# benjiebob/SMALify

Measured on AMD Instinct MI355X. Metric: fitter iterations/sec, higher is better.
Workload: dtype f32

## Files before the change

smalify_amd/csrc/kernels_lbs_backward.inc:

```

__global__ void __launch_bounds__(256)
vertex_bwd_kernel(ModelDev m, int M, const float* __restrict__ proj, const float* __restrict__ dface,
                  const float* __restrict__ dJ41 ,
                  const float* __restrict__ dverts_ext ,
                  const float* __restrict__ Am, float* __restrict__ dvert ,
                  float* __restrict__ dvp , float* __restrict__ dtr_part ) {
  __shared__ float As[420];
  __shared__ float dJs[123];
  __shared__ float red[16];
  const int Vp = m.Vp;
  PHASE_MARK(pv0);
  int n, vblock;
  xcd_block(Vp / 256, n, vblock);
  if (n >= M) return;
  const int v = vblock * 256 + threadIdx.x;
  constexpr int kPre = 8;
  const int vc = min(v, m.V - 1);
  const int vf0 = m.vf_off[vc], vf1 = (v < m.V) ? m.vf_off[vc + 1] : vf0;
  int vfi[kPre];
#pragma unroll
  for (int q = 0; q < kPre; ++q) vfi[q] = m.vf_idx[min(vf0 + q, max(vf1 - 1, vf0))];
  for (int i = threadIdx.x; i < 420; i += 256) As[i] = Am[(size_t)n * 420 + i];
  for (int i = threadIdx.x; i < 123; i += 256) dJs[i] = dJ41 ? dJ41[(size_t)n * 123 + i] : 0.f;
  __syncthreads();
// ... 110 lines not shown
  const int ncol = 3 * m.Vp;
  const int c = bx * 256 + threadIdx.x;
  float g = 0.f;
  if (c < ncol) {
    if (shared) {
      const int per = (M + gzn - 1) / gzn;
      const int n0 = bz * per, n1 = min(M, n0 + per);
      double gd = 0.0;
#pragma unroll 8
      for (int n = n0; n < n1; ++n) gd += (double)dvp[(size_t)n * ncol + c];
      g = (float)gd;
    } else {
      g = dvp[(size_t)by * ncol + c];
    }
  }
  const size_t pidx = (size_t)by * gzn * gx + (size_t)bz * gx + bx;
  const int lane = threadIdx.x & 63, w = threadIdx.x >> 6;
  for (int b0 = 0; b0 < nb; b0 += 32) {
    float val[32];
    const int cc = min(c, ncol - 1);
#pragma unroll
    for (int b = 0; b < 32; ++b) val[b] = m.sd[(size_t)min(b0 + b, nb - 1) * ncol + cc];
#pragma unroll
    for (int b = 0; b < 32; ++b) val[b] = (c < ncol && b0 + b < nb) ? g * val[b] : 0.f;
    const float tot = wave_sums<32>(val, lane);
    __syncthreads();
    if ((lane & 1) == 0) part[w][lane >> 1] = tot;
    __syncthreads();
    if (threadIdx.x < 32 && b0 + threadIdx.x < nb)
      dbeta_part[pidx * nb + b0 + threadIdx.x] = ((part[0][threadIdx.x] + part[1][threadIdx.x]) + part[2][threadIdx.x]) + part[3][threadIdx.x];
  }
}

constexpr int PBM_SPLITS = 24, PBM_U = 2, PBM_TILES = 4;
static_assert(PBM_SPLITS % 8 == 0, "the blocks of a column split are placed on one XCD (ids in chunks of 8 splits)");
__device__ __forceinline__ void
poseblend_bwd_mfma_block(const ModelDev& m, int M, int tchunk, int kpair, int split, const float* __restrict__ dvp,
                         float* __restrict__ dpf_part , float (*red)[8][64]) {
  const int lane = threadIdx.x & 63, w = threadIdx.x >> 6;
  const int ncol = 3 * m.Vp, nsteps = ncol / 16;
  const int per = (nsteps + PBM_SPLITS * 4 - 1) / (PBM_SPLITS * 4);
  const int s_beg = (split * 4 + w) * per, s_end = min(nsteps, s_beg + per);
  const int nft = (M + 15) / 16, t0 = tchunk * PBM_TILES, nt = min(PBM_TILES, nft - t0);
  const int k0 = kpair * 32;
  const int row = lane & 15, cq = (lane >> 4) * 4;
  const float4* pa[PBM_TILES];
#pragma unroll
  for (int t = 0; t < PBM_TILES; ++t)
    pa[t] = reinterpret_cast<const float4*>(dvp + (size_t)min((t0 + t) * 16 + row, M - 1) * ncol + cq);
  const float4* pb0 = reinterpret_cast<const float4*>(m.pd + (size_t)min(k0 + row, 305) * ncol + cq);
  const float4* pb1 = reinterpret_cast<const float4*>(m.pd + (size_t)min(k0 + 16 + row, 305) * ncol + cq);
  f32x4 acc0[PBM_TILES], acc1[PBM_TILES];
#pragma unroll
  for (int t = 0; t < PBM_TILES; ++t) { acc0[t] = f32x4{0.f, 0.f, 0.f, 0.f}; acc1[t] = acc0[t]; }
  for (int st0 = s_beg; st0 < s_end; st0 += PBM_U) {
    float4 B0[PBM_U], B1[PBM_U], A[PBM_TILES][PBM_U];
#pragma unroll
    for (int u = 0; u < PBM_U; ++u) {
      const int st = min(st0 + u, nsteps - 1);
      B0[u] = pb0[st * 4]; B1[u] = pb1[st * 4];
#pragma unroll
      for (int t = 0; t < PBM_TILES; ++t) {
        A[t][u] = make_float4(0.f, 0.f, 0.f, 0.f);
        if (t < nt && st0 + u < s_end) A[t][u] = pa[t][st * 4];
      }
    }
    __builtin_amdgcn_sched_barrier(0);
#pragma unroll
    for (int u = 0; u < PBM_U; ++u) {
#pragma unroll
      for (int t = 0; t < PBM_TILES; ++t) {
        if (t < nt) {
          acc0[t] = __builtin_amdgcn_mfma_f32_16x16x4f32(A[t][u].x, B0[u].x, acc0[t], 0, 0, 0);
          acc1[t] = __builtin_amdgcn_mfma_f32_16x16x4f32(A[t][u].x, B1[u].x, acc1[t], 0, 0, 0);
          acc0[t] = __builtin_amdgcn_mfma_f32_16x16x4f32(A[t][u].y, B0[u].y, acc0[t], 0, 0, 0);
          acc1[t] = __builtin_amdgcn_mfma_f32_16x16x4f32(A[t][u].y, B1[u].y, acc1[t], 0, 0, 0);
          acc0[t] = __builtin_amdgcn_mfma_f32_16x16x4f32(A[t][u].z, B0[u].z, acc0[t], 0, 0, 0);
          acc1[t] = __builtin_amdgcn_mfma_f32_16x16x4f32(A[t][u].z, B1[u].z, acc1[t], 0, 0, 0);
          acc0[t] = __builtin_amdgcn_mfma_f32_16x16x4f32(A[t][u].w, B0[u].w, acc0[t], 0, 0, 0);
          acc1[t] = __builtin_amdgcn_mfma_f32_16x16x4f32(A[t][u].w, B1[u].w, acc1[t], 0, 0, 0);
        }
      }
    }
    __builtin_amdgcn_sched_barrier(0);
  }
#pragma unroll
  for (int t = 0; t < PBM_TILES; ++t) {
    if (t < nt) {
#pragma unroll
      for (int r = 0; r < 4; ++r) { red[w][r][lane] = acc0[t][r]; red[w][4 + r][lane] = acc1[t][r]; }
      __syncthreads();
#pragma unroll
      for (int q = 0; q < 2; ++q) {
        const int reg = w * 2 + q, r = reg & 3, tile = reg >> 2;
        const float tot = ((red[0][reg][lane] + red[1][reg][lane]) + red[2][reg][lane]) + red[3][reg][lane];
        const int n = (t0 + t) * 16 + 4 * (lane >> 4) + r, k = k0 + tile * 16 + (lane & 15);
        if (n < M && k < 306) dpf_part[((size_t)split * M + n) * 308 + k] = tot;
      }
      __syncthreads();
    }
  }
}

__host__ __device__ inline int mid_pb_ids(int M) { return 10 * PBM_SPLITS * (((M + 15) / 16 + PBM_TILES - 1) / PBM_TILES); }
__host__ __device__ inline int mid_da_ids(int M) { return xcd_grid(35, M); }
__host__ __device__ inline int mid_grid(int M, int nPB) { return (nPB ? mid_pb_ids(M) : 0) + mid_da_ids(M); }
__global__ void __launch_bounds__(256, 4)
lbs_bwd_mid_kernel(ModelDev m, int M, int nPB, const float* __restrict__ dvert, const float* __restrict__ vposed,
                   const float* __restrict__ dvp, float* __restrict__ dA, float* __restrict__ dpf_part) {
  __shared__ float part[4][32];
  __shared__ float tile_red[4][8][64];
  int blk = blockIdx.x;
  if (nPB > 0) {
    const int ids = mid_pb_ids(M);
    if (blk < ids) {
      PHASE_MARK(pm0);
      const int tchunk = blk / (10 * PBM_SPLITS), r = blk - tchunk * (10 * PBM_SPLITS);
      const int chunk = r / 80, q = r - chunk * 80;
      poseblend_bwd_mfma_block(m, M, tchunk, q >> 3, chunk * 8 + (q & 7), dvp, dpf_part, tile_red);
      PHASE_MARK(pm1);
      PHASE_END(PH_MID_PB, pm0, pm1);
      return;
    }
    blk -= ids;
  }
  PHASE_MARK(pd0);
  int n, j;
  xcd_block_of(blk, 35, n, j);
  if (n >= M) return;
  dA_block(m, j, n, dvert, vposed, dA, part);
  PHASE_MARK(pd1); PHASE_END(PH_MID_DA, pd0, pd1);
}

__global__ void __launch_bounds__(256)
chain_bwd_kernel(ModelDev m, int M, const float* __restrict__ theta, const float* __restrict__ Rm,
                 const float* __restrict__ Gm, const float* __restrict__ scm,
                 const float* __restrict__ Jrest, int j_stride, const float* __restrict__ dA,
                 const float* __restrict__ dpf_part, int CS, const float* __restrict__ dth_direct,
                 float* __restrict__ dtheta , float* __restrict__ dls ,
                 float* __restrict__ dJrest , float* __restrict__ dbetaJ ,
                 float* __restrict__ dRs_out ,
                 int nb, int betas_shared, int nDB_x, int nDB_y, int nDB_z, const float* __restrict__ dvp,
                 float* __restrict__ dbeta_part ) {
  PHASE_MARK(pc0);
  if ((int)blockIdx.x >= M) {
    __shared__ float rpart[4][32];
    const int blk = (int)blockIdx.x - M;
    dbeta_block(m, M, nb, betas_shared, blk % nDB_x, (blk / nDB_x) % nDB_y, blk / (nDB_x * nDB_y), nDB_x, nDB_z, dvp, dbeta_part, rpart);
    PHASE_MARK(pcr);
    PHASE_END(PH_CHAIN_RIDER, pc0, pcr);
    return;
  }
  __shared__ float R[35][9], G[35][12], sc[35][3], J[35][3];
  __shared__ float dG[35][12], dR[35][9], dJ[35][3];
  __shared__ float cG[35][12], cJ[35][3], cS[35][3], sOwn[35][3];
  __shared__ float dRp[35][9], djv[35][3];
  __shared__ int sidx[105];
  __shared__ float psum[4][320];
  __shared__ float isc[35][3];
  __shared__ float sJS[105 * 48];
  __shared__ float dAs[35][12];
  __shared__ unsigned char t_lvl_off[36], t_lvl_joint[36], t_child_off[36], t_child_idx[36], t_par[36];
  __shared__ uint2 t_sch[kTreeMaxPass][8];
  const int n = blockIdx.x, l = threadIdx.x;
  const TreeLevels& tl = m.tree;
  if (l < 36) {
    t_lvl_off[l] = tl.lvl_off[l]; t_child_off[l] = tl.child_off[l];
    if (l < 35) { t_lvl_joint[l] = tl.lvl_joint[l]; t_child_idx[l] = tl.child_idx[l]; t_par[l] = (unsigned char)max(m.parents[l], 0); }
  }
  if (l >= 128 && l < 128 + kTreeMaxPass * 8) {
    const int q = l - 128;
    const unsigned char* ch = tl.pass_child[q >> 3][q & 7];
    t_sch[q >> 3][q & 7] = make_uint2((unsigned)tl.pass_joint[q >> 3][q & 7] | ((unsigned)tl.pass_parent[q >> 3][q & 7] << 8) | ((unsigned)tl.pass_nchild[q >> 3][q & 7] << 16),
                                      (unsigned)ch[0] | ((unsigned)ch[1] << 8) | ((unsigned)ch[2] << 16) | ((unsigned)ch[3] << 24));
  }
  const int lth = min(l, 34);
  const float th_pre[3] = {theta[((size_t)n * 35 + lth) * 3], theta[((size_t)n * 35 + lth) * 3 + 1], theta[((size_t)n * 35 + lth) * 3 + 2]};
  float dthd_pre[3] = {0.f, 0.f, 0.f};
  if (dth_direct) {
#pragma unroll
    for (int a = 0; a < 3; ++a) dthd_pre[a] = dth_direct[(size_t)n * 105 + lth * 3 + a];
  }
  const int nlev = tl.nlev;
  const bool js_lds = dbetaJ && m.NBall <= 48;
  const int njs = js_lds ? 105 * m.NBall : 1;
  float js_tmp[20];
  const float* js_src = js_lds ? m.JS : Rm + (size_t)n * 315;
#pragma unroll
  for (int r = 0; r < 20; ++r) js_tmp[r] = js_src[min(l + 256 * r, njs - 1)];
  {
    const int l2 = l + 256;
    const float r0v = Rm[(size_t)n * 315 + l], r1v = Rm[(size_t)n * 315 + min(l2, 314)];
    const float g0v = Gm[(size_t)n * 420 + l], g1v = Gm[(size_t)n * 420 + min(l2, 419)];
    const float a0v = dA[(size_t)n * 420 + l], a1v = dA[(size_t)n * 420 + min(l2, 419)];
    const int lc = min(l, 104);
    const float sv = scm[(size_t)n * 105 + lc], jv = Jrest[(size_t)n * j_stride + lc];
    const int siv = m.scale_idx[lc];
    constexpr int kMaxPer = (PBM_SPLITS + 3) / 4;
    const int per = (CS + 3) / 4, qd = l >> 6, c0 = qd * per, c1 = min(CS, c0 + per);
    const size_t stride = (size_t)M * 308;
    float pv[5][kMaxPer];
    const bool fast = dpf_part != nullptr && per <= kMaxPer;
    if (fast) {
#pragma unroll
      for (int r = 0; r < 5; ++r) {
        const float* src = dpf_part + (size_t)n * 308 + min((l & 63) + 64 * r, 305);
#pragma unroll
        for (int c = 0; c < kMaxPer; ++c) pv[r][c] = src[(size_t)min(c0 + c, CS - 1) * stride];
      }
    }
    if (js_lds) {
#pragma unroll
      for (int r = 0; r < 20; ++r) { const int i = l + 256 * r; if (i < njs) sJS[i] = js_tmp[r]; }
    }
    R[l / 9][l % 9] = r0v;
    if (l2 < 315) R[l2 / 9][l2 % 9] = r1v;
    G[l / 12][l % 12] = g0v; dAs[l / 12][l % 12] = a0v;
    if (l2 < 420) { G[l2 / 12][l2 % 12] = g1v; dAs[l2 / 12][l2 % 12] = a1v; }
    if (l < 105) {
      sc[l / 3][l % 3] = sv; isc[l / 3][l % 3] = 1.0f / sv;
      J[l / 3][l % 3] = jv;
      sOwn[l / 3][l % 3] = 0.f; cS[l / 3][l % 3] = 0.f; cJ[l / 3][l % 3] = 0.f;
      sidx[l] = siv;
    }
    if (dpf_part) {
#pragma unroll
      for (int r = 0; r < 5; ++r) {
        const int el = (l & 63) + 64 * r;
        if (el < 306) {
          float sacc = 0.f;
          if (fast) {
            if (c0 < c1) sacc = pv[r][0];
#pragma unroll
            for (int c = 1; c < kMaxPer; ++c)
              if (c0 + c < c1) sacc += pv[r][c];
          } else {
            const float* src = dpf_part + (size_t)n * 308 + el;
            for (int c = c0; c < c1; ++c) sacc += src[c * stride];
          }
          psum[qd][el] = sacc;
        }
      }
    }
  }
  __syncthreads();
  PHASE_MARK(pc1);
  for (int i = l; i < 315; i += 256)
    dR[i / 9][i % 9] = (i >= 9 && dpf_part) ? ((psum[0][i - 9] + psum[1][i - 9]) + psum[2][i - 9]) + psum[3][i - 9] : 0.f;
  for (int i = l; i < 420; i += 256) {
    const int j = i / 12, e = i % 12, a = e >> 2, b = e & 3;
    const float* da = dAs[j];
    dG[j][e] = (b < 3) ? da[e] - da[a * 4 + 3] * J[j][b] : da[e];
  }
  for (int i = l; i < 105; i += 256) {
    const int j = i / 3, c = i % 3;
    const float* da = dAs[j];
    dJ[j][c] = -(G[j][0 * 4 + c] * da[3] + G[j][1 * 4 + c] * da[7] + G[j][2 * 4 + c] * da[11]);
  }
  __syncthreads();
  PHASE_MARK(pc2);
  const int slot = l / 12, e = l % 12;
  if (l < 64 && tl.fast) {
    const int npass = tl.npass;
    const int slot_c = min(slot, 7);
    uint2 sch_n = t_sch[max(npass - 1, 0)][slot_c];
#pragma unroll 1
    for (int k = npass - 1; k >= 0; --k) {
      const uint2 sch = sch_n;
      sch_n = t_sch[max(k - 1, 0)][slot_c];
      const bool live = (sch.x & 255u) != 255u;
      const int i = live ? (int)(sch.x & 255u) : 0, p = live ? (int)((sch.x >> 8) & 255u) : 0, nch = live ? (int)(sch.x >> 16) : 0;
      const unsigned chil_k = sch.y;
      if (live) {
        float acc = dG[i][e];
        float cv[kTreeMaxChildren];
#pragma unroll
        for (int q = 0; q < kTreeMaxChildren; ++q) cv[q] = cG[(chil_k >> (8 * q)) & 255u][e];
#pragma unroll
        for (int q = 0; q < kTreeMaxChildren; ++q) acc += (q < nch) ? cv[q] : 0.f;
        dG[i][e] = acc;
      }
      __builtin_amdgcn_fence(__ATOMIC_ACQ_REL, "wavefront");
      __builtin_amdgcn_wave_barrier();
      if (live) {
        if (e < 9) {
          const int a = e / 3, b = e % 3;
          dRp[i][e] = G[p][0 * 4 + a] * dG[i][0 * 4 + b] + G[p][1 * 4 + a] * dG[i][1 * 4 + b] + G[p][2 * 4 + a] * dG[i][2 * 4 + b];
        } else {
          const int a = e - 9;
          djv[i][a] = G[p][0 * 4 + a] * dG[i][3] + G[p][1 * 4 + a] * dG[i][7] + G[p][2 * 4 + a] * dG[i][11];
        }
      }
      __builtin_amdgcn_fence(__ATOMIC_ACQ_REL, "wavefront");
      __builtin_amdgcn_wave_barrier();
      if (live) {
        if (e < 9) {
          const int a = e / 3, c = e % 3;
          float acc = dG[i][a * 4 + 3] * (J[i][c] - J[p][c]);
#pragma unroll
          for (int b = 0; b < 3; ++b) acc = fmaf(dG[i][a * 4 + b], R[i][c * 3 + b] * sc[i][b] * isc[p][c], acc);
          cG[i][a * 4 + c] = acc;
          dR[i][a * 3 + c] += dRp[i][a * 3 + c] * sc[i][c] * isc[p][a];
        } else {
          const int a = e - 9;
          cG[i][a * 4 + 3] = dG[i][a * 4 + 3];
          cJ[i][a] = djv[i][a];
          {
            const int b = a;
            float acc = 0.f;
#pragma unroll
            for (int r = 0; r < 3; ++r) acc = fmaf(dRp[i][r * 3 + b], R[i][r * 3 + b] * isc[p][r], acc);
            sOwn[i][b] = acc;
          }
          {
            float acc = 0.f;
#pragma unroll
            for (int b = 0; b < 3; ++b) acc = fmaf(dRp[i][a * 3 + b], R[i][a * 3 + b] * sc[i][b] * isc[p][a], acc);
            cS[i][a] = acc * isc[p][a];
          }
        }
      }
      __builtin_amdgcn_fence(__ATOMIC_ACQ_REL, "wavefront");
      __builtin_amdgcn_wave_barrier();
    }
  } else if (l < 64)
  for (int L = nlev - 1; L >= 1; --L) {
    const int j0 = t_lvl_off[L], nj = t_lvl_off[L + 1] - j0;
    for (int base = 0; base < nj; base += 5) {
      const bool live = (slot < 5) && (base + slot < nj);
      const int i = live ? t_lvl_joint[j0 + base + slot] : 0;
      const int p = live ? t_par[i] : 0;
      if (live) {
        float acc = dG[i][e];
        for (int q = t_child_off[i]; q < t_child_off[i + 1]; ++q) acc += cG[t_child_idx[q]][e];
        dG[i][e] = acc;
      }
      __builtin_amdgcn_fence(__ATOMIC_ACQ_REL, "workgroup");
      __builtin_amdgcn_wave_barrier();
      if (live) {
        if (e < 9) {
          const int a = e / 3, b = e % 3;
          dRp[i][e] = G[p][0 * 4 + a] * dG[i][0 * 4 + b] + G[p][1 * 4 + a] * dG[i][1 * 4 + b] + G[p][2 * 4 + a] * dG[i][2 * 4 + b];
        } else {
          const int a = e - 9;
          djv[i][a] = G[p][0 * 4 + a] * dG[i][3] + G[p][1 * 4 + a] * dG[i][7] + G[p][2 * 4 + a] * dG[i][11];
        }
      }
      __builtin_amdgcn_fence(__ATOMIC_ACQ_REL, "workgroup");
      __builtin_amdgcn_wave_barrier();
      if (live) {
        if (e < 9) {
          const int a = e / 3, c = e % 3;
          float acc = dG[i][a * 4 + 3] * (J[i][c] - J[p][c]);
#pragma unroll
          for (int b = 0; b < 3; ++b) acc = fmaf(dG[i][a * 4 + b], R[i][c * 3 + b] * sc[i][b] * isc[p][c], acc);
          cG[i][a * 4 + c] = acc;
          dR[i][a * 3 + c] += dRp[i][a * 3 + c] * sc[i][c] * isc[p][a];
        } else {
          const int a = e - 9;
          cG[i][a * 4 + 3] = dG[i][a * 4 + 3];
          cJ[i][a] = djv[i][a];
          {
            const int b = a;
            float acc = 0.f;
#pragma unroll
            for (int r = 0; r < 3; ++r) acc = fmaf(dRp[i][r * 3 + b], R[i][r * 3 + b] * isc[p][r], acc);
            sOwn[i][b] = acc;
          }
          {
            float acc = 0.f;
#pragma unroll
            for (int b = 0; b < 3; ++b) acc = fmaf(dRp[i][a * 3 + b], R[i][a * 3 + b] * sc[i][b] * isc[p][a], acc);
            cS[i][a] = acc * isc[p][a];
          }
        }
      }
      __builtin_amdgcn_fence(__ATOMIC_ACQ_REL, "workgroup");
      __builtin_amdgcn_wave_barrier();
    }
  }
  __syncthreads();
  PHASE_MARK(pc3);
  if (l < 12) {
    float acc = dG[0][l];
    for (int q = t_child_off[0]; q < t_child_off[1]; ++q) acc += cG[t_child_idx[q]][l];
    dG[0][l] = acc;
  }
  __syncthreads();
  if (l < 9) dR[0][l] += dG[0][(l / 3) * 4 + (l % 3)];
  for (int i = l; i < 105; i += 256) {
    const int j = i / 3, a = i % 3;
    float aj = dJ[j][a], as = 0.f;
    for (int q = t_child_off[j]; q < t_child_off[j + 1]; ++q) { aj -= cJ[t_child_idx[q]][a]; as -= cS[t_child_idx[q]][a]; }
    if (j > 0) { aj += cJ[j][a]; as += sOwn[j][a]; }
    else aj += dG[0][a * 4 + 3];
    dJ[j][a] = aj;
    sOwn[j][a] = as;
  }
  __syncthreads();
  PHASE_MARK(pc4);
  if (l < 35) {
    const float th[3] = {th_pre[0], th_pre[1], th_pre[2]};
    float g[9], d[3];
#pragma unroll
    for (int q = 0; q < 9; ++q) g[q] = dR[l][q];
    if (dRs_out) {
#pragma unroll
      for (int q = 0; q < 9; ++q) dRs_out[((size_t)n * 35 + l) * 9 + q] = g[q];
    }
    rodrigues_bwd(th, g, d);
#pragma unroll
    for (int a = 0; a < 3; ++a)
      dtheta[(size_t)n * 105 + l * 3 + a] = d[a] + (dth_direct ? dthd_pre[a] : 0.f);
  }
  if (dls) {
    const int w = l >> 6, lane = l & 63;
    for (int sidx_l = w; sidx_l < 6; sidx_l += 4) {
      float v = 0.f;
      if (sidx[lane] == sidx_l) v = sOwn[lane / 3][lane % 3] * sc[lane / 3][lane % 3];
      if (lane + 64 < 105 && sidx[lane + 64] == sidx_l) v += sOwn[(lane + 64) / 3][(lane + 64) % 3] * sc[(lane + 64) / 3][(lane + 64) % 3];
      v = wave_sum(v);
      if (lane == 0) dls[(size_t)n * 6 + sidx_l] = v;
    }
  }
  for (int i = l; i < 105; i += 256) dJrest[(size_t)n * 105 + i] = dJ[i / 3][i % 3];
  if (dbetaJ) {
    const int w = l >> 6, b = l & 63;
    if (b < m.NBall) {
      float acc = 0.f;
      if (js_lds) {
#pragma unroll 9
        for (int r = 0; r < 27; ++r) { const int i = w * 27 + r; if (i < 105) acc = fmaf(dJ[i / 3][i % 3], sJS[i * m.NBall + b], acc); }
      } else {
        for (int i = w * 27; i < min(105, w * 27 + 27); ++i) acc = fmaf(dJ[i / 3][i % 3], m.JS[i * m.NBall + b], acc);
      }
      psum[w][b] = acc;
    }
    __syncthreads();
    if (l < m.NBall) dbetaJ[(size_t)n * m.NBall + l] = ((psum[0][l] + psum[1][l]) + psum[2][l]) + psum[3][l];
  }
  PHASE_MARK(pc5);
  PHASE_ADD(PH_CHAIN, 0, pc0, pc1); PHASE_ADD(PH_CHAIN, 1, pc1, pc2); PHASE_ADD(PH_CHAIN, 2, pc2, pc3); PHASE_ADD(PH_CHAIN, 3, pc3, pc4); PHASE_ADD(PH_CHAIN, 4, pc4, pc5);
  PHASE_END(PH_CHAIN, pc0, pc5);
}

template <bool kPerImage>
__global__ void __launch_bounds__(256)
assemble_kernel(AssembleArgs a, AssembleExt x) {
  __shared__ float red[16];
  __shared__ double bsum[12][32];
  __shared__ float part[32][8];
  __shared__ double dpart[32][8];
  __shared__ int is_last;
  const int t = threadIdx.x;
  PHASE_MARK(pa0);
  const int M = a.M;
  const int nbs = a.betas_shared ? 1 : M;
  int role = blockIdx.x;
  const int ph_role = (role < nbs) ? PH_ASM_BETA : PH_ASM_ELEM;
  if (role < nbs) {
    if (a.g_betas) {
      const int s = role;
      for (int b0 = 0; b0 < a.nb; b0 += 20) {
        if (b0) __syncthreads();
        BetaOperands bo;
        asm_beta_fetch(a, s, b0, bo);
        asm_beta_slices(a, s, b0, bo, bsum);
        __syncthreads();
        const float tot = asm_beta_total(a, s, b0, bo, bsum);
        if constexpr (kPerImage) {
          if (t < 20 && b0 + t < a.nb) a.g_betas[s * a.nb + b0 + t] = x.gb_prior_pf ? tot + x.gb_prior_pf[(size_t)s * x.gb_stride + b0 + t] : tot;
        } else
        if (t < 20 && b0 + t < a.nb) a.g_betas[s * a.nb + b0 + t] = tot;
      }
    }
  } else if ((role -= nbs) == 0) {
    if (a.g_ls) {
      if (a.ls_shared) {
        LsOperands lo;
        asm_ls_fetch(a, lo);
        asm_ls_slices(a, lo, dpart);
        __syncthreads();
        const float tot = asm_ls_total(a, lo, dpart);
        if (t < 6) a.g_ls[t] = tot;
      } else {
        if (kPerImage && x.gls_prior_pf)
          for (int i = t; i < M * 6; i += 256) a.g_ls[i] = a.dls[i] + x.gls_prior_pf[(size_t)(i / 6) * x.gls_stride + i % 6];
        else
          for (int i = t; i < M * 6; i += 256) a.g_ls[i] = a.dls[i];
      }
    }
  } else if ((role -= 1) < kAsmElem) {
    const int gt = role * 256 + t, gs = kAsmElem * 256;
    for (int i = gt; i < M * 3; i += gs) {
      const int n = i / 3, e = i % 3;
      if (a.g_grot) a.g_grot[i] = asm_grot_elem(a, n, e);
      if (a.g_trans) a.g_trans[i] = asm_trans_elem(a, n, e);
    }
    if (a.g_jrot) {
      const int total = M * 102;
      for (int i0 = gt; i0 < total; i0 += 8 * gs) {
        float v[8];
#pragma unroll
        for (int u = 0; u < 8; ++u) {
          const int i = min(i0 + u * gs, total - 1), n = i / 102, e = i % 102;
          v[u] = asm_jrot_elem(a, n, e);
        }
#pragma unroll
        for (int u = 0; u < 8; ++u)
          if (i0 + u * gs < total) a.g_jrot[i0 + u * gs] = v[u];
      }
    }
  } else if (a.losses) {
    role -= kAsmElem;
    float lsil = 0.f;
    if (a.tile_loss) {
      for (int k = role * 256 + t; k < M * a.T; k += kAsmLoss * 256) {
        const int n = k / a.T;
        const int Bn = frame_window_size(n, a.win);
        lsil += a.tile_loss[k] * (a.w_sil / ((float)Bn * (float)a.S * (float)a.S));
      }
    }
    long long qs = 0;
    if (a.qloss) for (int k = role * 256 + t; k < a.nqblk; k += kAsmLoss * 256) qs += a.qloss[k];
    qs = wave_sum_i64(qs);
    __shared__ long long qred[4];
    if ((t & 63) == 0) qred[t >> 6] = qs;
    lsil = block_sum(lsil, red);
    if (t == 0) { a.lpart[role] = lsil; a.qpart[role] = (qred[0] + qred[1]) + (qred[2] + qred[3]); }
  }
  PHASE_MARK(pa1);
  PHASE_END(ph_role, pa0, pa1);
  (void)ph_role;
  if (!a.losses) return;
  __threadfence();
  __syncthreads();
  if (t == 0) is_last = (atomicAdd(a.counter, 1) == (int)gridDim.x - 1);
  __syncthreads();
  if (!is_last) return;
  __threadfence();
  static_assert(kAsmLoss == 16, "butterfly below");
  float lsil = 0.f;
  if (t < 64) {
    const volatile float* lp = a.lpart;
    lsil = (t < kAsmLoss) ? lp[t] : 0.f;
#pragma unroll
    for (int o = 8; o > 0; o >>= 1) lsil += __shfl_xor(lsil, o, 64);
// ... 262 lines not shown
```

smalify_amd/csrc/kernels_lbs_forward.inc:

```

constexpr int kAsmFr = 8, kAsmPa = 32, kAsmLs = 4;
struct BetaOperands { float fv[kAsmFr], pv[kAsmPa], prior; };
__device__ __forceinline__ void asm_beta_fetch(const AssembleArgs& a, int s, int b0, BetaOperands& o) {
  const int t = threadIdx.x, slice = min(t / 20, 11), b = min(b0 + t % 20, a.nb - 1);
  const int nlo = a.betas_shared ? 0 : s, nhi = a.betas_shared ? a.M : s + 1, nparts = a.nblk_beta * a.ngrp_beta;
  const float* pj = a.dbetaJ + b;
  const float* pp = a.dbeta_part + (size_t)s * nparts * a.nb + b;
#pragma unroll
  for (int u = 0; u < kAsmFr; ++u) o.fv[u] = pj[(size_t)min(nlo + slice + 12 * u, nhi - 1) * a.NBall];
#pragma unroll
  for (int u = 0; u < kAsmPa; ++u) o.pv[u] = pp[(size_t)min(slice + 12 * u, nparts - 1) * a.nb];
  o.prior = (a.gb_prior && s == 0) ? a.gb_prior[min(b0 + min(t, 19), a.nb - 1)] : 0.f;
}
__device__ __forceinline__ void asm_beta_slices(const AssembleArgs& a, int s, int b0, BetaOperands& o, double (*bsum)[32]) {
  const int t = threadIdx.x, bl = t % 20, slice = t / 20, b = b0 + bl;
  if (slice < 12 && b < a.nb) {
    const int nlo = a.betas_shared ? 0 : s, nhi = a.betas_shared ? a.M : s + 1, nparts = a.nblk_beta * a.ngrp_beta;
    const float* pj = a.dbetaJ + b;
    const float* pp = a.dbeta_part + (size_t)s * nparts * a.nb + b;
    double acc = 0.0;
    for (int n0 = nlo + slice; n0 < nhi; n0 += 12 * kAsmFr) {
#pragma unroll
      for (int u = 0; u < kAsmFr; ++u)
        if (n0 + 12 * u < nhi) acc += (double)o.fv[u];
// ... 56 lines not shown
}
__device__ __forceinline__ float asm_theta_elem(const AssembleArgs& a, int n, int l) {
  const float* mk = (l < 3) ? a.gmask + l : a.rmask + max(l - 3, 0);
  return a.dtheta[(size_t)n * 105 + l] * *mk;
}
__device__ __forceinline__ float asm_grot_elem(const AssembleArgs& a, int n, int e) { return asm_theta_elem(a, n, e); }
__device__ __forceinline__ float asm_jrot_elem(const AssembleArgs& a, int n, int e) { return asm_theta_elem(a, n, 3 + e); }
__device__ __forceinline__ float asm_trans_elem(const AssembleArgs& a, int n, int e) {
  double acc = a.dtr_direct ? (double)a.dtr_direct[n * 3 + e] : 0.0;
#pragma unroll 16
  for (int vt = 0; vt < a.nvt; ++vt) acc += (double)a.dtr_part[((size_t)vt * a.M + n) * 3 + e];
  return (float)acc;
}


struct HeadArgs {
  int M, Mp, nb, betas_stride, ls_stride, nshape_x, nshape, prior_D, prior_use_ls;
  const float* betas;
  const float* theta_in;
  const float* grot;
  const float* jrot;
  const float* gmask;
  const float* rmask;
  const float* logscale;
  float* theta;
  float* Jrest;
  float* v_shaped;
  float *Rm, *Gm, *scm, *Am, *pfT;
  const float* prior_prec;
  const float* prior_mean;
  float prior_w;
  float *prior_loss, *prior_gb, *prior_gls;
  const float* Rs_in;
  const float* joff;
  int joff_stride;
  const float* voff;
};

constexpr int kPendingNb = 20;
struct HeadShared {
  float beta[kPendingNb], ls[8], grot[4];
  double bsum[12][32], dpart[32][8];
};
struct AdamOperands { float p, m, v; };
__device__ __forceinline__ AdamOperands pending_load(const PendingStep& p, const PendingTensor& T, int i) {
  return AdamOperands{T.p_in[i], p.fresh ? 0.f : T.m_in[i], p.fresh ? 0.f : T.v_in[i]};
}
__device__ __forceinline__ float pending_adam(const PendingStep& p, const PendingTensor& T, int i, const AdamOperands& o, float gi, bool store) {
  float mi, vi, pv = o.p;
  adam_update(gi, o.m, o.v, p.b1, p.b2, p.eps, p.step_size, p.bc2_sqrt, mi, vi, pv);
  if (store) { T.m[i] = mi; T.v[i] = vi; T.p[i] = pv; T.g[i] = gi; }
  return pv;
}
struct SharedOperands { AdamOperands beta, ls; BetaOperands bo; LsOperands lo; };
__device__ __forceinline__ void pending_shared_fetch(const PendingStep& p, const HeadArgs& a, int n, SharedOperands& o) {
  const int t = threadIdx.x;
  o.beta = pending_load(p, p.betas, min(t, 19));
  if (p.betas.train) asm_beta_fetch(p.g, 0, 0, o.bo);
  if (a.logscale) {
    if (p.g.ls_shared) o.ls = pending_load(p, p.ls, min(t, 5));
    else if (!p.ls.train) o.ls.p = a.logscale[(size_t)n * a.ls_stride + min(t, 5)];
    if (p.ls.train && p.g.ls_shared) asm_ls_fetch(p.g, o.lo);
  }
}
__device__ __forceinline__ void pending_shared_slices(const PendingStep& p, SharedOperands& o, HeadShared& sh) {
  if (p.betas.train) asm_beta_slices(p.g, 0, 0, o.bo, sh.bsum);
  if (p.ls.train && p.g.ls_shared) asm_ls_slices(p.g, o.lo, sh.dpart);
}
__device__ __forceinline__ void pending_shared_step(const PendingStep& p, const HeadArgs& a, const SharedOperands& o, HeadShared& sh) {
  const int t = threadIdx.x;
  const bool store = blockIdx.x == 0;
  if (p.betas.train) {
    const float gi = asm_beta_total(p.g, 0, 0, o.bo, sh.bsum);
    if (t < 20) sh.beta[t] = pending_adam(p, p.betas, t, o.beta, gi, store);
  } else if (t < 20) {
    sh.beta[t] = o.beta.p;
  }
  if (a.logscale && (p.g.ls_shared || !p.ls.train)) {
    if (p.ls.train) {
      const float gi = asm_ls_total(p.g, o.lo, sh.dpart);
      if (t < 6) sh.ls[t] = pending_adam(p, p.ls, t, o.ls, gi, store);
    } else if (t < 6) {
      sh.ls[t] = o.ls.p;
    }
  }
}
struct ThetaOperands { AdamOperands ao; float gi; };
__device__ __forceinline__ void pending_jrot_fetch(const PendingStep& p, int n, ThetaOperands& o) {
  const int l = max(min((int)threadIdx.x, 104), 3);
  o.ao = pending_load(p, p.jrot, n * 102 + (l - 3));
  o.gi = asm_theta_elem(p.g, n, l);
}
__device__ __forceinline__ float pending_jrot_step(const PendingStep& p, int n, const ThetaOperands& o) {
  const int l = threadIdx.x;
  if (l >= 3 && l < 105 && p.jrot.train) return pending_adam(p, p.jrot, n * 102 + (l - 3), o.ao, o.gi, true);
  return o.ao.p;
}
__device__ __forceinline__ void pending_frame_extras(const PendingStep& p, int n, HeadShared& sh) {
  const int l = threadIdx.x;
  if (l >= 128 && l < 131) {
    const int i = n * 3 + (l - 128);
    if (p.trans.train) pending_adam(p, p.trans, i, pending_load(p, p.trans, i), asm_trans_elem(p.g, n, l - 128), true);
  } else if (l >= 224 && l < 227) {
    const int i = n * 3 + (l - 224);
    const AdamOperands ao = pending_load(p, p.grot, i);
    sh.grot[l - 224] = p.grot.train ? pending_adam(p, p.grot, i, ao, asm_theta_elem(p.g, n, l - 224), true) : ao.p;
  } else if (l >= 192 && l < 198) {
    if (p.ls.train && !p.g.ls_shared) { const int i = n * 6 + (l - 192); sh.ls[l - 192] = pending_adam(p, p.ls, i, pending_load(p, p.ls, i), p.g.dls[i], true); }
  }
}

template <bool kPending>
__device__ __forceinline__ void
pose_block(const ModelDev& m, const HeadArgs& a, int n, const PendingStep* pend, HeadShared* sh) {
  __shared__ float th[105];
  __shared__ float R[35][9];
  __shared__ float sc[35][3], isc[35][3];
  __shared__ __attribute__((aligned(16))) float G[35][12];
  __shared__ float J[35][3];
  __shared__ unsigned char t_lvl_off[36], t_lvl_joint[36], t_par[36];
  __shared__ unsigned char t_pj[kTreeMaxPass][8], t_pp[kTreeMaxPass][8];
  const int l = threadIdx.x, M = a.M;
  PHASE_MARK(ph0);
  const TreeLevels& tl = m.tree;
  if (l < 36) {
    t_lvl_off[l] = tl.lvl_off[l];
    if (l < 35) { t_lvl_joint[l] = tl.lvl_joint[l]; t_par[l] = (unsigned char)max(m.parents[l], 0); }
  }
  if (l >= 128 && l < 128 + kTreeMaxPass * 8) { const int q = l - 128; t_pj[q >> 3][q & 7] = tl.pass_joint[q >> 3][q & 7]; t_pp[q >> 3][q & 7] = tl.pass_parent[q >> 3][q & 7]; }
  const int nlev = tl.nlev;
  float tv_pend = 0.f, js_pre[kPendingNb], jt_pre = 0.f, mv_pre = 0.f;
  int idx_pre = 0;
  if constexpr (kPending) {
    const int lc = min(l, 104);
    idx_pre = m.scale_idx[lc]; jt_pre = m.Jt[lc];
    mv_pre = (lc < 3) ? a.gmask[lc] : a.rmask[max(lc - 3, 0)];
#pragma unroll
    for (int b = 0; b < kPendingNb; ++b) js_pre[b] = m.JS[lc * m.NBall + b];
    SharedOperands so;
    ThetaOperands to;
    pending_shared_fetch(*pend, a, n, so);
    pending_jrot_fetch(*pend, n, to);
    pending_frame_extras(*pend, n, *sh);
    tv_pend = pending_jrot_step(*pend, n, to);
    pending_shared_slices(*pend, so, *sh);
    PHASE_MARK(pp1);
    __syncthreads();
    pending_shared_step(*pend, a, so, *sh);
    PHASE_MARK(pp2);
    __syncthreads();
    if (l < 3) tv_pend = sh->grot[l];
    PHASE_MARK(pp3);
    PHASE_ADD(PH_HEAD_POSE, 4, ph0, pp1); PHASE_ADD(PH_HEAD_POSE, 5, pp1, pp2); PHASE_ADD(PH_HEAD_POSE, 6, pp2, pp3);
  }
  if (l < 105) {
    const int lj = max(l - 3, 0);
    const float* tsrc = a.theta_in ? a.theta_in + (size_t)n * 105 + l : ((l < 3) ? a.grot + n * 3 + l : a.jrot + (size_t)n * 102 + lj);
    const float* msrc = a.theta_in ? tsrc : ((l < 3) ? a.gmask + l : a.rmask + lj);
    int idx;
    float tv0, mv, lsv, acc;
    if constexpr (kPending) {
      idx = idx_pre; tv0 = tv_pend; mv = mv_pre; acc = jt_pre;
      lsv = a.logscale ? sh->ls[max(idx, 0)] : 0.f;
    } else {
      idx = m.scale_idx[l];
      tv0 = *tsrc; mv = *msrc;
      acc = m.Jt[l];
      lsv = a.logscale ? a.logscale[(size_t)n * a.ls_stride + max(idx, 0)] : 0.f;
    }
    const float tv = a.theta_in ? tv0 : tv0 * mv;
    th[l] = tv;
    a.theta[(size_t)n * 105 + l] = tv;
    if constexpr (kPending) {
#pragma unroll
      for (int b = 0; b < kPendingNb; ++b) acc = fmaf(js_pre[b], sh->beta[b], acc);
    } else {
      const float* beta = a.betas + (size_t)(a.betas_stride ? n : 0) * a.betas_stride;
#pragma unroll 10
      for (int b = 0; b < a.nb; ++b) acc = fmaf(m.JS[l * m.NBall + b], beta[b], acc);
    }
    if (a.joff) acc += a.joff[(size_t)n * a.joff_stride + l];
    J[l / 3][l % 3] = acc;
    if (a.betas_stride || n == 0) a.Jrest[(size_t)(a.betas_stride ? n : 0) * 105 + l] = acc;
    const float sv = (a.logscale != nullptr && idx >= 0) ? expf(lsv) : 1.0f;
    sc[l / 3][l % 3] = sv; isc[l / 3][l % 3] = 1.0f / sv;
    a.scm[(size_t)n * 105 + l] = sv;
  }
  __syncthreads();
  PHASE_MARK(ph1);
  if (l < 35) {
    const float t3[3] = {th[l * 3], th[l * 3 + 1], th[l * 3 + 2]};
    float r[9];
    if (a.Rs_in) {
#pragma unroll
      for (int e = 0; e < 9; ++e) r[e] = a.Rs_in[((size_t)n * 35 + l) * 9 + e];
    } else {
      rodrigues_fwd(t3, r);
    }
#pragma unroll
    for (int e = 0; e < 9; ++e) { R[l][e] = r[e]; a.Rm[((size_t)n * 35 + l) * 9 + e] = r[e]; }
  }
  __syncthreads();
  PHASE_MARK(ph2);
  for (int idx = l; idx < 306; idx += 256) {
    const int j = idx / 9 + 1, e = idx % 9;
    a.pfT[(size_t)idx * a.Mp + n] = R[j][e] - ((e & 3) == 0 ? 1.0f : 0.0f);
  }
  if (l < 12) {
    const int r = l >> 2, c = l & 3;
    G[0][l] = (c < 3) ? R[0][r * 3 + c] : J[0][r];
  }
  if (l < 64 && tl.fast) {
    const int slot_c = min(l / 12, 7), e = l % 12, r = e >> 2, c = e & 3, cc = min(c, 2);
    const int npass = tl.npass;
    auto fetch = [&](int k, int& ijp, float (&kc)[3]) {
      const int i = t_pj[k][slot_c], p = t_pp[k][slot_c];
      const bool live = i != 255;
      ijp = live ? (i | (p << 8)) : -1;
      const int ii = live ? i : 0;
#pragma unroll
      for (int q = 0; q < 3; ++q) {
        const float rot = R[ii][q * 3 + cc] * sc[ii][cc] * isc[p][q], dj = J[ii][q] - J[p][q];
        kc[q] = (c < 3) ? rot : dj;
      }
    };
    int ijp_n;
    float kc_n[3];
    fetch(0, ijp_n, kc_n);
#pragma unroll 1
    for (int k = 0; k < npass; ++k) {
      const int ijp = ijp_n;
      const float k0 = kc_n[0], k1 = kc_n[1], k2 = kc_n[2];
      fetch(min(k + 1, kTreeMaxPass - 1), ijp_n, kc_n);
      __builtin_amdgcn_fence(__ATOMIC_ACQ_REL, "wavefront");
      __builtin_amdgcn_wave_barrier();
      if (ijp >= 0) {
        const int i = ijp & 255, p = ijp >> 8;
        const float4 g = *reinterpret_cast<const float4*>(&G[p][r * 4]);
        float acc = (c < 3) ? 0.f : g.w;
        acc = fmaf(g.x, k0, acc);
        acc = fmaf(g.y, k1, acc);
        acc = fmaf(g.z, k2, acc);
        G[i][e] = acc;
      }
    }
  } else if (l < 64) {
    const int slot = l / 12, e = l % 12;
    for (int L = 1; L < nlev; ++L) {
      const int j0 = t_lvl_off[L], nj = t_lvl_off[L + 1] - j0;
      for (int base = 0; base < nj; base += 5) {
        __builtin_amdgcn_fence(__ATOMIC_ACQ_REL, "workgroup");
        __builtin_amdgcn_wave_barrier();
        if (slot < 5 && base + slot < nj) {
          const int i = t_lvl_joint[j0 + base + slot], p = t_par[i];
          const int r = e >> 2, c = e & 3;
          float acc;
          if (c < 3) {
            acc = 0.f;
#pragma unroll
            for (int q = 0; q < 3; ++q) acc = fmaf(G[p][r * 4 + q], R[i][q * 3 + c] * sc[i][c] * isc[p][q], acc);
          } else {
            acc = G[p][r * 4 + 3];
#pragma unroll
            for (int q = 0; q < 3; ++q) acc = fmaf(G[p][r * 4 + q], J[i][q] - J[p][q], acc);
          }
          G[i][e] = acc;
        }
      }
    }
  }
  __syncthreads();
  PHASE_MARK(ph3);
  for (int idx = l; idx < 35 * 12; idx += 256) {
    const int j = idx / 12, e = idx % 12, r = e >> 2, c = e & 3;
    float val = G[j][e];
    if (c == 3) {
#pragma unroll
      for (int q = 0; q < 3; ++q) val = fmaf(-G[j][r * 4 + q], J[j][q], val);
    }
    a.Am[(size_t)n * 420 + idx] = val;
    a.Gm[(size_t)n * 420 + idx] = G[j][e];
  }
  (void)M;
  PHASE_MARK(ph4);
  PHASE_ADD(PH_HEAD_POSE, 0, ph0, ph1); PHASE_ADD(PH_HEAD_POSE, 1, ph1, ph2); PHASE_ADD(PH_HEAD_POSE, 2, ph2, ph3); PHASE_ADD(PH_HEAD_POSE, 3, ph3, ph4);
  PHASE_END(PH_HEAD_POSE, ph0, ph4);
}

constexpr int kPriorFrames = 16;
struct PriorFrames {
  int on, gb_stride, gls_stride;
  float* loss;
  float *gb, *gls;
};
__device__ __forceinline__ void prior_frames_block(const HeadArgs& a, const PriorFrames& pf, int pb) {
  __shared__ float prec[26 * 26], mean[32], xs[4][32], rs[4][32];
  const int t = threadIdx.x, lane = t & 63, w = t >> 6, D = a.prior_D;
  for (int i = t; i < D * D; i += 256) prec[i] = a.prior_prec[i];
  if (t < D) mean[t] = a.prior_mean[t];
  __syncthreads();
  const int n_end = min((pb + 1) * kPriorFrames, a.M);
  for (int n = pb * kPriorFrames + w; n < n_end; n += 4) {
    if (lane < D)
      xs[w][lane] = ((lane < 20) ? a.betas[(size_t)n * a.betas_stride + lane] : a.logscale[(size_t)n * a.ls_stride + lane - 20]) - mean[lane];
    __builtin_amdgcn_fence(__ATOMIC_ACQ_REL, "workgroup");
    __builtin_amdgcn_wave_barrier();
// ... 679 lines not shown
```

smalify_amd/csrc/smalfit_kernels.hip:

```cpp
#include <hip/hip_runtime.h>
#include <stdint.h>

#include "smalfit_internal.h"
#include "mesh3d_math.h"
#include "smalfit_plan.h"

namespace smalfit {

__device__ __forceinline__ float wave_sum(float v) {
#pragma unroll
  for (int o = 32; o > 0; o >>= 1) v += __shfl_xor(v, o, 64);
  return v;
}

__device__ __forceinline__ float block_sum(float v, float* red ) {
  v = wave_sum(v);
  const int w = threadIdx.x >> 6, nw = blockDim.x >> 6;
  __syncthreads();
  if ((threadIdx.x & 63) == 0) red[w] = v;
  __syncthreads();
  float t = 0.f;
  for (int i = 0; i < nw; ++i) t += red[i];
  return t;
}

template <int HALF>
__device__ __forceinline__ void fold_accumulators(float* acc, int lane, int bit) {
#pragma unroll
  for (int j = 0; j < HALF; ++j) {
    const bool up = (lane & bit) != 0;
    const float keep = up ? acc[HALF + j] : acc[j];
    const float send = up ? acc[j] : acc[HALF + j];
    acc[j] = keep + __shfl_xor(send, bit, 64);
  }
}

template <int NV>
__device__ __forceinline__ float wave_sums(float* v, int lane) {
  static_assert(NV == 16 || NV == 32, "16 or 32 values");
  fold_accumulators<NV / 2>(v, lane, 32);
  fold_accumulators<NV / 4>(v, lane, 16);
  fold_accumulators<NV / 8>(v, lane, 8);
  fold_accumulators<NV / 16>(v, lane, 4);
  if (NV == 32) fold_accumulators<NV / 32>(v, lane, 2);
  float r = v[0];
  if (NV == 16) r += __shfl_xor(r, 2, 64);
  r += __shfl_xor(r, 1, 64);
  return r;
}

__device__ __forceinline__ int frame_window_size(int n, const WinMap& w) {
  const int start = ((n + w.offset) / w.window) * w.window;
  const int rem = w.total - start;
  return rem < w.window ? rem : w.window;
}

#ifdef SMALFIT_PHASES
__device__ unsigned long long g_phase[12][16];
#define PHASE_MARK(var) const unsigned long long var = __builtin_amdgcn_s_memtime()
#define PHASE_ADD(k, i, t0, t1) do { if (threadIdx.x == 0) atomicAdd(&g_phase[k][i], (t1) - (t0)); } while (0)
#define PHASE_END(k, t0, t1) do { if (threadIdx.x == 0) { atomicAdd(&g_phase[k][15], 1ull); atomicMax(&g_phase[k][14], (t1) - (t0)); atomicAdd(&g_phase[k][13], (t1) - (t0)); } } while (0)
#else
#define PHASE_MARK(var)
#define PHASE_ADD(k, i, t0, t1)
#define PHASE_END(k, t0, t1)
#endif
enum { PH_HEAD_POSE = 0, PH_HEAD_SHAPE, PH_SKIN, PH_VERTEX_BWD, PH_MID_PB, PH_MID_DA, PH_CHAIN, PH_CHAIN_RIDER, PH_ASM_BETA, PH_ASM_ELEM, PH_ASM_LAST, PH_ADAM };

#include "kernels_lbs_forward.inc"
#include "kernels_raster.inc"
#include "kernels_color.inc"
#include "kernels_lbs_backward.inc"
#include "kernels_mesh3d.inc"

}

#include "smalfit_launch.inc"
#include "smalfit_mesh3d.inc"
```

Measured before the change: 2944.

## Shorten serial tree backward pass by hoisting per-joint rotation terms out of chain

The sequential per-level loop of the kinematic-chain backward pass now does only the child-gradient accumulation and the propagated cG term. It prefetches the per-joint coefficient constants one pass ahead and reads dG/cG rows as float4 vectors. The dRp, dR, sOwn and cS computations, which do not feed the serial dependency, move into block-parallel loops after the tree walk, and the cJ/djv arrays are folded into extra dRp columns. This cuts the work and wavefront barriers on the latency-bound serial path, at the cost of an extra __syncthreads and some redundant reads afterward. A per-thread phase timing macro is also added, and it only compiles in when profiling is enabled.

```diff
diff --git a/smalify_amd/csrc/kernels_lbs_backward.inc b/smalify_amd/csrc/kernels_lbs_backward.inc
--- a/smalify_amd/csrc/kernels_lbs_backward.inc
+++ b/smalify_amd/csrc/kernels_lbs_backward.inc
@@ -286,9 +286,10 @@
     return;
   }
   __shared__ float R[35][9], G[35][12], sc[35][3], J[35][3];
-  __shared__ float dG[35][12], dR[35][9], dJ[35][3];
-  __shared__ float cG[35][12], cJ[35][3], cS[35][3], sOwn[35][3];
-  __shared__ float dRp[35][9], djv[35][3];
+  __shared__ float dR[35][9], dJ[35][3];
+  __shared__ __attribute__((aligned(16))) float dG[35][12], cG[35][12];
+  __shared__ float cS[35][3], sOwn[35][3];
+  __shared__ float dRp[35][12];
   __shared__ int sidx[105];
   __shared__ float psum[4][320];
   __shared__ float isc[35][3];
@@ -354,7 +355,7 @@
     if (l < 105) {
       sc[l / 3][l % 3] = sv; isc[l / 3][l % 3] = 1.0f / sv;
       J[l / 3][l % 3] = jv;
-      sOwn[l / 3][l % 3] = 0.f; cS[l / 3][l % 3] = 0.f; cJ[l / 3][l % 3] = 0.f;
+      sOwn[l / 3][l % 3] = 0.f; cS[l / 3][l % 3] = 0.f; dRp[l / 3][9 + l % 3] = 0.f;
       sidx[l] = siv;
     }
     if (dpf_part) {
@@ -394,66 +395,45 @@
   __syncthreads();
   PHASE_MARK(pc2);
   const int slot = l / 12, e = l % 12;
+  const bool rot = e < 9;
+  const int ea = rot ? e / 3 : e - 9, ec = rot ? e % 3 : 0, eo = rot ? ea * 4 + ec : ea * 4 + 3;
   if (l < 64 && tl.fast) {
     const int npass = tl.npass;
     const int slot_c = min(slot, 7);
-    uint2 sch_n = t_sch[max(npass - 1, 0)][slot_c];
+    auto fetch = [&](int k, uint2& sch, float (&kc)[4]) {
+      sch = t_sch[k][slot_c];
+      const bool live = (sch.x & 255u) != 255u;
+      const int i = live ? (int)(sch.x & 255u) : 0, p = live ? (int)((sch.x >> 8) & 255u) : 0;
+#pragma unroll
+      for (int b = 0; b < 3; ++b) kc[b] = R[i][ec * 3 + b] * sc[i][b] * isc[p][ec];
+      kc[3] = J[i][ec] - J[p][ec];
+    };
+    uint2 sch_n;
+    float kc_n[4];
+    fetch(max(npass - 1, 0), sch_n, kc_n);
 #pragma unroll 1
     for (int k = npass - 1; k >= 0; --k) {
       const uint2 sch = sch_n;
-      sch_n = t_sch[max(k - 1, 0)][slot_c];
+      const float k0 = kc_n[0], k1 = kc_n[1], k2 = kc_n[2], k3 = kc_n[3];
+      fetch(max(k - 1, 0), sch_n, kc_n);
       const bool live = (sch.x & 255u) != 255u;
-      const int i = live ? (int)(sch.x & 255u) : 0, p = live ? (int)((sch.x >> 8) & 255u) : 0, nch = live ? (int)(sch.x >> 16) : 0;
+      const int i = live ? (int)(sch.x & 255u) : 0, nch = live ? (int)(sch.x >> 16) : 0;
       const unsigned chil_k = sch.y;
-      if (live) {
-        float acc = dG[i][e];
-        float cv[kTreeMaxChildren];
-#pragma unroll
-        for (int q = 0; q < kTreeMaxChildren; ++q) cv[q] = cG[(chil_k >> (8 * q)) & 255u][e];
-#pragma unroll
-        for (int q = 0; q < kTreeMaxChildren; ++q) acc += (q < nch) ? cv[q] : 0.f;
-        dG[i][e] = acc;
-      }
-      __builtin_amdgcn_fence(__ATOMIC_ACQ_REL, "wavefront");
-      __builtin_amdgcn_wave_barrier();
-      if (live) {
-        if (e < 9) {
-          const int a = e / 3, b = e % 3;
-          dRp[i][e] = G[p][0 * 4 + a] * dG[i][0 * 4 + b] + G[p][1 * 4 + a] * dG[i][1 * 4 + b] + G[p][2 * 4 + a] * dG[i][2 * 4 + b];
-        } else {
-          const int a = e - 9;
-          djv[i][a] = G[p][0 * 4 + a] * dG[i][3] + G[p][1 * 4 + a] * dG[i][7] + G[p][2 * 4 + a] * dG[i][11];
-        }
-      }
-      __builtin_amdgcn_fence(__ATOMIC_ACQ_REL, "wavefront");
-      __builtin_amdgcn_wave_barrier();
-      if (live) {
-        if (e < 9) {
-          const int a = e / 3, c = e % 3;
-          float acc = dG[i][a * 4 + 3] * (J[i][c] - J[p][c]);
-#pragma unroll
-          for (int b = 0; b < 3; ++b) acc = fmaf(dG[i][a * 4 + b], R[i][c * 3 + b] * sc[i][b] * isc[p][c], acc);
-          cG[i][a * 4 + c] = acc;
-          dR[i][a * 3 + c] += dRp[i][a * 3 + c] * sc[i][c] * isc[p][a];
-        } else {
-          const int a = e - 9;
-          cG[i][a * 4 + 3] = dG[i][a * 4 + 3];
-          cJ[i][a] = djv[i][a];
-          {
-            const int b = a;
-            float acc = 0.f;
-#pragma unroll
-            for (int r = 0; r < 3; ++r) acc = fmaf(dRp[i][r * 3 + b], R[i][r * 3 + b] * isc[p][r], acc);
-            sOwn[i][b] = acc;
-          }
-          {
-            float acc = 0.f;
-#pragma unroll
-            for (int b = 0; b < 3; ++b) acc = fmaf(dRp[i][a * 3 + b], R[i][a * 3 + b] * sc[i][b] * isc[p][a], acc);
-            cS[i][a] = acc * isc[p][a];
-          }
-        }
-      }
+      float4 row = *reinterpret_cast<const float4*>(&dG[i][ea * 4]);
+      float4 cv[kTreeMaxChildren];
+#pragma unroll
+      for (int q = 0; q < kTreeMaxChildren; ++q) cv[q] = *reinterpret_cast<const float4*>(&cG[(chil_k >> (8 * q)) & 255u][ea * 4]);
+#pragma unroll
+      for (int q = 0; q < kTreeMaxChildren; ++q) {
+        row.x += (q < nch) ? cv[q].x : 0.f; row.y += (q < nch) ? cv[q].y : 0.f;
+        row.z += (q < nch) ? cv[q].z : 0.f; row.w += (q < nch) ? cv[q].w : 0.f;
+      }
+      float acc = row.w * k3;
+      acc = fmaf(row.x, k0, acc);
+      acc = fmaf(row.y, k1, acc);
+      acc = fmaf(row.z, k2, acc);
+      const float own = rot ? (ec == 0 ? row.x : ec == 1 ? row.y : row.z) : row.w;
+      if (live) { dG[i][eo] = own; cG[i][eo] = rot ? acc : row.w; }
       __builtin_amdgcn_fence(__ATOMIC_ACQ_REL, "wavefront");
       __builtin_amdgcn_wave_barrier();
     }
@@ -472,41 +452,13 @@
       __builtin_amdgcn_fence(__ATOMIC_ACQ_REL, "workgroup");
       __builtin_amdgcn_wave_barrier();
       if (live) {
-        if (e < 9) {
-          const int a = e / 3, b = e % 3;
-          dRp[i][e] = G[p][0 * 4 + a] * dG[i][0 * 4 + b] + G[p][1 * 4 + a] * dG[i][1 * 4 + b] + G[p][2 * 4 + a] * dG[i][2 * 4 + b];
+        if (rot) {
+          float acc = dG[i][ea * 4 + 3] * (J[i][ec] - J[p][ec]);
+#pragma unroll
+          for (int b = 0; b < 3; ++b) acc = fmaf(dG[i][ea * 4 + b], R[i][ec * 3 + b] * sc[i][b] * isc[p][ec], acc);
+          cG[i][eo] = acc;
         } else {
-          const int a = e - 9;
-          djv[i][a] = G[p][0 * 4 + a] * dG[i][3] + G[p][1 * 4 + a] * dG[i][7] + G[p][2 * 4 + a] * dG[i][11];
-        }
-      }
-      __builtin_amdgcn_fence(__ATOMIC_ACQ_REL, "workgroup");
-      __builtin_amdgcn_wave_barrier();
-      if (live) {
-        if (e < 9) {
-          const int a = e / 3, c = e % 3;
-          float acc = dG[i][a * 4 + 3] * (J[i][c] - J[p][c]);
-#pragma unroll
-          for (int b = 0; b < 3; ++b) acc = fmaf(dG[i][a * 4 + b], R[i][c * 3 + b] * sc[i][b] * isc[p][c], acc);
-          cG[i][a * 4 + c] = acc;
-          dR[i][a * 3 + c] += dRp[i][a * 3 + c] * sc[i][c] * isc[p][a];
-        } else {
-          const int a = e - 9;
-          cG[i][a * 4 + 3] = dG[i][a * 4 + 3];
-          cJ[i][a] = djv[i][a];
-          {
-            const int b = a;
-            float acc = 0.f;
-#pragma unroll
-            for (int r = 0; r < 3; ++r) acc = fmaf(dRp[i][r * 3 + b], R[i][r * 3 + b] * isc[p][r], acc);
-            sOwn[i][b] = acc;
-          }
-          {
-            float acc = 0.f;
-#pragma unroll
-            for (int b = 0; b < 3; ++b) acc = fmaf(dRp[i][a * 3 + b], R[i][a * 3 + b] * sc[i][b] * isc[p][a], acc);
-            cS[i][a] = acc * isc[p][a];
-          }
+          cG[i][eo] = dG[i][eo];
         }
       }
       __builtin_amdgcn_fence(__ATOMIC_ACQ_REL, "workgroup");
@@ -520,13 +472,39 @@
     for (int q = t_child_off[0]; q < t_child_off[1]; ++q) acc += cG[t_child_idx[q]][l];
     dG[0][l] = acc;
   }
+  for (int idx = l; idx < 34 * 12; idx += 256) {
+    const int i = idx / 12 + 1, q = idx % 12, p = t_par[i];
+    const int a = q < 9 ? q / 3 : q - 9, b = q < 9 ? q % 3 : 3;
+    dRp[i][q] = G[p][0 * 4 + a] * dG[i][0 * 4 + b] + G[p][1 * 4 + a] * dG[i][1 * 4 + b] + G[p][2 * 4 + a] * dG[i][2 * 4 + b];
+  }
   __syncthreads();
   if (l < 9) dR[0][l] += dG[0][(l / 3) * 4 + (l % 3)];
+  for (int idx = l; idx < 34 * 9; idx += 256) {
+    const int i = idx / 9 + 1, q = idx % 9, a = q / 3, c = q % 3, p = t_par[i];
+    dR[i][a * 3 + c] += dRp[i][a * 3 + c] * sc[i][c] * isc[p][a];
+  }
+  if (l >= 128 && l < 128 + 34 * 3) {
+    const int i = (l - 128) / 3 + 1, a = (l - 128) % 3, p = t_par[i];
+    {
+      const int b = a;
+      float acc = 0.f;
+#pragma unroll
+      for (int r = 0; r < 3; ++r) acc = fmaf(dRp[i][r * 3 + b], R[i][r * 3 + b] * isc[p][r], acc);
+      sOwn[i][b] = acc;
+    }
+    {
+      float acc = 0.f;
+#pragma unroll
+      for (int b = 0; b < 3; ++b) acc = fmaf(dRp[i][a * 3 + b], R[i][a * 3 + b] * sc[i][b] * isc[p][a], acc);
+      cS[i][a] = acc * isc[p][a];
+    }
+  }
+  __syncthreads();
   for (int i = l; i < 105; i += 256) {
     const int j = i / 3, a = i % 3;
     float aj = dJ[j][a], as = 0.f;
-    for (int q = t_child_off[j]; q < t_child_off[j + 1]; ++q) { aj -= cJ[t_child_idx[q]][a]; as -= cS[t_child_idx[q]][a]; }
-    if (j > 0) { aj += cJ[j][a]; as += sOwn[j][a]; }
+    for (int q = t_child_off[j]; q < t_child_off[j + 1]; ++q) { aj -= dRp[t_child_idx[q]][9 + a]; as -= cS[t_child_idx[q]][a]; }
+    if (j > 0) { aj += dRp[j][9 + a]; as += sOwn[j][a]; }
     else aj += dG[0][a * 4 + 3];
     dJ[j][a] = aj;
     sOwn[j][a] = as;
diff --git a/smalify_amd/csrc/kernels_lbs_forward.inc b/smalify_amd/csrc/kernels_lbs_forward.inc
--- a/smalify_amd/csrc/kernels_lbs_forward.inc
+++ b/smalify_amd/csrc/kernels_lbs_forward.inc
@@ -232,6 +232,7 @@
     if (l < 3) tv_pend = sh->grot[l];
     PHASE_MARK(pp3);
     PHASE_ADD(PH_HEAD_POSE, 4, ph0, pp1); PHASE_ADD(PH_HEAD_POSE, 5, pp1, pp2); PHASE_ADD(PH_HEAD_POSE, 6, pp2, pp3);
+    PHASE_ADD_AT(PH_HEAD_POSE, 7, ph0, pp1, 128); PHASE_ADD_AT(PH_HEAD_POSE, 8, ph0, pp1, 192);
   }
   if (l < 105) {
     const int lj = max(l - 3, 0);
diff --git a/smalify_amd/csrc/smalfit_kernels.hip b/smalify_amd/csrc/smalfit_kernels.hip
--- a/smalify_amd/csrc/smalfit_kernels.hip
+++ b/smalify_amd/csrc/smalfit_kernels.hip
@@ -59,10 +59,12 @@
 __device__ unsigned long long g_phase[12][16];
 #define PHASE_MARK(var) const unsigned long long var = __builtin_amdgcn_s_memtime()
 #define PHASE_ADD(k, i, t0, t1) do { if (threadIdx.x == 0) atomicAdd(&g_phase[k][i], (t1) - (t0)); } while (0)
+#define PHASE_ADD_AT(k, i, t0, t1, tid) do { if (threadIdx.x == (tid)) atomicAdd(&g_phase[k][i], (t1) - (t0)); } while (0)
 #define PHASE_END(k, t0, t1) do { if (threadIdx.x == 0) { atomicAdd(&g_phase[k][15], 1ull); atomicMax(&g_phase[k][14], (t1) - (t0)); atomicAdd(&g_phase[k][13], (t1) - (t0)); } } while (0)
 #else
 #define PHASE_MARK(var)
 #define PHASE_ADD(k, i, t0, t1)
+#define PHASE_ADD_AT(k, i, t0, t1, tid)
 #define PHASE_END(k, t0, t1)
 #endif
 enum { PH_HEAD_POSE = 0, PH_HEAD_SHAPE, PH_SKIN, PH_VERTEX_BWD, PH_MID_PB, PH_MID_DA, PH_CHAIN, PH_CHAIN_RIDER, PH_ASM_BETA, PH_ASM_ELEM, PH_ASM_LAST, PH_ADAM };
```

Result: no change. 2968, median of 6 (+0.8%).
